# SafeRL-Lab/Massive-MARL-Benchmark

Hardware: AMD Instinct MI355X
Metric: env-steps/sec (whole node), TenAnt 4096 envs/GPU, PPO rollout (higher is better)
Workload: dtype f32 (policy-layer products: fp32 operands as 2 row-scaled fp16 planes (kept to 2^-22), 3 f16 MFMA products, fp32 accumulation; error vs float64 <= the exact-fp32 MFMA kernel's, see policy_layers_error_vs_f64); 1 GPU; TenAnt num_envs=4096 per GPU, PPO rollout: ActorCritic MLP [1024,1024,512]x2 (fp32) + fused sim step (dt 0.0166, 2 substeps) + RolloutStorage + GAE every 8 steps; envs_per_gpu=4096, global_envs=4096, parallelism=env-sharded x1, no data-path collective, hipgraph=True, refresh_in_graph=True, rollouts_per_graph=1, fused_act_and_bound_slots=True, obs_planes_from_step_kernel=True, policy_head_in_step_kernel=True, critic_stream=True, critic_deferred=False, finite=True, resets_total=97569

## Files before the change

include/mms.h:

```cpp
#ifndef MMS_H
#define MMS_H

#include <stdint.h>

#ifdef __cplusplus
extern "C" {
#endif

#define MMS_ABI_VERSION 4
#define MMS_DR_FLOATS 33

enum mms_task { MMS_TASK_TEN_ANT = 0, MMS_TASK_ONE_ANT = 1, MMS_TASK_MULTI_INGENUITY = 2,
                MMS_TASK_MULTI_ANT_CIRCLE = 3 };
enum mms_dtype { MMS_F32 = 0, MMS_I64 = 1, MMS_I32 = 2, MMS_U8 = 3 };

typedef struct mms_model {
    float torso_mass, torso_ixx, torso_izz, torso_radius;
    float leg_mass, leg_ia, leg_it;
    float foot_mass, foot_ia, foot_it;
    float limb_radius, leg_len, foot_len;
    float hip_pos[4][3];
    float limb_dir[4][3];
    float ankle_axis[4][3];
    float dof_lower[8], dof_upper[8], dof_init[8], gear[8];
// ... 176 lines not shown
#define MMS_H32_BYTES(rows, K) ((size_t)(rows) * (size_t)(((K) + 31) / 32) * 128)

int mms_split_planes16_group(int device, int32_t groups, int64_t rows, int32_t K, int32_t x_pitch, const float* const* x, void* const* planes,
                             float* const* scale, float* const* inv, int32_t nchains, int32_t L, const float* const* chain,
                             float* const* chain_scale, float* const* chain_inv, float* const* stat, float eps, void* hip_stream);

int mms_split_planes16_cat(int device, int64_t rows, int32_t K0, int32_t pitch0, const float* x0, int32_t K1, int32_t pitch1, const float* x1,
                           void* planes, float* scale, float* inv, int32_t nchains, int32_t L, const float* chain, float* chain_scale,
                           float* chain_inv, void* hip_stream);

int mms_weight_planes16_group(int device, int32_t groups, const int64_t* N, const int32_t* K, const float* const* w, void* const* planes,
                              float* const* scale, float* const* inv, float* const* l1, void* hip_stream);
int mms_chain_refresh16(int device, int32_t nchains, int32_t L, const float* const* l1, const float* const* bias, const int32_t* n,
                        float* chain, float bound0, int64_t rows, float* chain_scale, float* chain_inv, void* hip_stream);

int mms_linear_group_act_split16(int device, int32_t groups, int64_t M, int32_t N, int32_t K, const void* const* x, const void* const* w,
                                 const float* const* b, void* const* y, const float* const* x_inv, const float* const* w_inv,
                                 const float* const* y_scale, int32_t act, int32_t out_mode, const float* const* ln_s,
                                 const float* const* ln_stat_in, float* const* ln_part_out, const float* const* head_w, float* const* head_part,
                                 const int32_t* head_dims, void* hip_stream);

int mms_fold_planes16_group(int device, int32_t groups, const int64_t* N, const int32_t* K, const float* const* w, const float* const* gamma,
                            const float* const* beta, const float* const* bias, void* const* planes, float* const* inv, float* const* s,
                            float* const* c, float* const* rb, float* const* wt, void* hip_stream);
int mms_fold_scales16_group(int device, int32_t groups, const float* const* rb, const int32_t* n, int64_t M, float* const* scale1,
                            float* const* ysc, float* const* yinv, void* hip_stream);

int mms_row_stats_chan_group(int device, int32_t groups, int64_t M, int32_t slots, const float* const* part, float* const* stat, float eps,
                             void* hip_stream);

// ... 53 lines not shown
```

massive_marl_benchmark_amd/_lib.py:

```python
import ctypes
import os

from .model import MmsConfig, MmsTensor

_HERE = os.path.dirname(os.path.abspath(__file__))
LIB_PATH = os.environ.get("MMS_LIB", os.path.join(_HERE, "lib", "libmms.so"))
LIB_CPU_PATH = os.path.join(_HERE, "lib", "libmms_cpu.so")
_lib = None
_lib_cpu = None

SYMBOLS = ["mms_create", "mms_destroy", "mms_get_tensor", "mms_step", "mms_post_step", "mms_reset_all", "mms_set_state",
           "mms_bind_obs_out", "mms_bind_obs_planes16", "mms_bind_actions", "mms_bind_policy_head", "mms_set_dr", "mms_set_obs_outputs", "mms_bind_rollout_out", "mms_ppo_act", "mms_ppo_heads_act", "mms_sac_heads_act", "mms_q_heads_backup", "mms_det_heads_act_group", "mms_q_heads_backup_group", "mms_linear2_act", "mms_linear_group_act", "mms_split_planes", "mms_split_planes_group", "mms_linear_group_act_split", "mms_split_planes16_group", "mms_split_planes16_cat", "mms_weight_planes16_group", "mms_chain_refresh16", "mms_fold_planes16_group", "mms_fold_scales16_group", "mms_linear_group_act_split16", "mms_row_stats_chan_group", "mms_marl_heads_finish", "mms_row_stats_group", "mms_row_moments_group", "mms_layernorm_group", "mms_marl_heads_act", "mms_marl_views", "mms_gae_ppo", "mms_adv_normalize", "mms_gae_ppo_normalized", "mms_layer_clock_probe", "mms_gae_marl", "mms_gae_marl_agents", "mms_mlp_grad", "mms_mlp_grad_rop", "mms_ln_mlp_grad", "mms_ln_mlp_jvp", "mms_ppo_loss", "mms_marl_ppo_loss",
           "mms_last_error", "mms_abi_version"]


class MmsError(RuntimeError):
    pass


def _bind(path):
    L = ctypes.CDLL(path)
    vp, ci, c64, cf = ctypes.c_void_p, ctypes.c_int, ctypes.c_int64, ctypes.c_float
    L.mms_create.argtypes = [ctypes.POINTER(MmsConfig), ctypes.POINTER(vp)]
    L.mms_destroy.argtypes = [vp]
    L.mms_get_tensor.argtypes = [vp, ctypes.c_char_p, ctypes.POINTER(MmsTensor)]
    L.mms_step.argtypes = [vp, vp]
    L.mms_post_step.argtypes = [vp, vp]
# ... 14 lines not shown
    L.mms_q_heads_backup.argtypes = [ci, c64, ctypes.c_int32, vp, vp, vp, vp, vp, vp, vp, vp, vp, vp, vp, cf, cf, vp, vp]
    L.mms_det_heads_act_group.argtypes = [ci, ctypes.c_int32, c64, ctypes.c_int32, ctypes.c_int32, ctypes.c_int32, vp, vp, vp, vp, cf, ctypes.c_uint64, vp, c64, vp, c64, vp, c64, vp]
    L.mms_q_heads_backup_group.argtypes = [ci, ctypes.c_int32, c64, ctypes.c_int32, vp, vp, vp, vp, vp, vp, cf, vp, vp]
    L.mms_linear2_act.argtypes = [ci, c64, ctypes.c_int32, ctypes.c_int32, vp, vp, vp, vp, vp, vp, vp, vp, ctypes.c_int32, vp]
    L.mms_linear_group_act.argtypes = [ci, ctypes.c_int32, c64, ctypes.c_int32, ctypes.c_int32, vp, vp, vp, vp, ctypes.c_int32, vp, vp, vp, vp]
    L.mms_split_planes.argtypes = [ci, c64, ctypes.c_int32, ctypes.c_int32, vp, vp, vp]
    L.mms_split_planes_group.argtypes = [ci, ctypes.c_int32, c64, ctypes.c_int32, ctypes.c_int32, vp, vp, vp]
    L.mms_linear_group_act_split.argtypes = [ci, ctypes.c_int32, c64, ctypes.c_int32, ctypes.c_int32, vp, vp, vp, vp, ctypes.c_int32, ctypes.c_int32,
                                             vp, vp, vp, vp, vp, vp, vp]
    L.mms_split_planes16_group.argtypes = [ci, ctypes.c_int32, c64, ctypes.c_int32, ctypes.c_int32, vp, vp, vp, vp, ctypes.c_int32, ctypes.c_int32, vp, vp, vp, vp, cf, vp]
    L.mms_split_planes16_cat.argtypes = [ci, c64, ctypes.c_int32, ctypes.c_int32, vp, ctypes.c_int32, ctypes.c_int32, vp, vp, vp, vp, ctypes.c_int32, ctypes.c_int32, vp, vp, vp, vp]
    L.mms_weight_planes16_group.argtypes = [ci, ctypes.c_int32, vp, vp, vp, vp, vp, vp, vp, vp]
    L.mms_fold_planes16_group.argtypes = [ci, ctypes.c_int32, vp, vp, vp, vp, vp, vp, vp, vp, vp, vp, vp, vp, vp]
    L.mms_fold_scales16_group.argtypes = [ci, ctypes.c_int32, vp, vp, c64, vp, vp, vp, vp]
    L.mms_chain_refresh16.argtypes = [ci, ctypes.c_int32, ctypes.c_int32, vp, vp, vp, vp, cf, c64, vp, vp, vp]
    L.mms_linear_group_act_split16.argtypes = [ci, ctypes.c_int32, c64, ctypes.c_int32, ctypes.c_int32, vp, vp, vp, vp, vp, vp, vp, ctypes.c_int32, ctypes.c_int32,
                                               vp, vp, vp, vp, vp, vp, vp]
    L.mms_row_stats_chan_group.argtypes = [ci, ctypes.c_int32, c64, ctypes.c_int32, vp, vp, cf, vp]
    L.mms_marl_heads_finish.argtypes = [ci, ctypes.c_int32, c64, ctypes.c_int32, vp, vp, vp, vp, vp, vp, vp, vp, vp, vp, ctypes.c_uint64, c64, cf, vp]
    L.mms_row_moments_group.argtypes = [ci, ctypes.c_int32, c64, ctypes.c_int32, ctypes.c_int32, vp, vp, cf, vp]
    L.mms_row_stats_group.argtypes = [ci, ctypes.c_int32, c64, ctypes.c_int32, ctypes.c_int32, vp, vp, cf, vp]
    L.mms_layernorm_group.argtypes = [ci, ctypes.c_int32, c64, ctypes.c_int32, ctypes.c_int32, ctypes.c_int32, vp, vp, vp, vp, cf, vp]
    L.mms_marl_heads_act.argtypes = [ci, ctypes.c_int32, c64, ctypes.c_int32, vp, vp, vp, vp, vp, vp, vp, vp, vp, vp, vp, ctypes.c_uint64, c64, cf, vp]
    L.mms_marl_views.argtypes = [ci, vp, vp, c64, ctypes.c_int32, ctypes.c_int32, ctypes.c_int32, vp]
    L.mms_gae_ppo.argtypes = [ci, vp, vp, vp, vp, vp, vp, vp, ctypes.c_int32, c64, cf, cf, vp]
    L.mms_adv_normalize.argtypes = [ci, vp, vp, c64, vp]
    L.mms_gae_ppo_normalized.argtypes = [ci, vp, vp, vp, vp, vp, vp, vp, ctypes.c_int32, c64, cf, cf, vp]
    L.mms_layer_clock_probe.argtypes = [ci, vp, ctypes.c_int32]
    L.mms_gae_marl.argtypes = [ci, vp, vp, vp, vp, ctypes.c_int32, c64, cf, cf, ctypes.c_int32, vp, vp, vp]
    L.mms_gae_marl_agents.argtypes = [ci, vp, vp, vp, vp, ctypes.c_int32, c64, ctypes.c_int32, cf, cf, ctypes.c_int32, vp, vp, vp]
# ... 54 lines not shown
```

massive_marl_benchmark_amd/algorithms/rl/ppo/module.py:

```python
import ctypes
import math

import numpy as np
import torch
import torch.nn as nn

from .... import _lib


def get_activation(act_name):
    table = {"elu": nn.ELU, "selu": nn.SELU, "relu": nn.ReLU, "crelu": nn.ReLU, "lrelu": nn.LeakyReLU, "tanh": nn.Tanh,
             "sigmoid": nn.Sigmoid}
    if act_name not in table:
        print("invalid activation function!")
        return None
    return table[act_name]()


def _mlp(in_dim, hidden, out_dim, activation):
    layers, d = [], in_dim
    for h in hidden:
        layers += [nn.Linear(d, h), activation]
        d = h
    layers.append(nn.Linear(d, out_dim))
# ... 164 lines not shown
    def _chain(self, st, members):
        o0, Lh = st["slices"][members[0]]
        if Lh == 0:
            return None, 0
        for j, g in enumerate(members):
            assert st["slices"][g] == (o0 + 2 * Lh * j, Lh), "networks that share an input must be adjacent and equally deep"
        return st["bounds"][o0: o0 + 2 * Lh * len(members)], Lh

    def refresh(self):
        dev = self.log_std.device
        vers, addrs = self._param_tags()
        if self._addr_tag is not None and self._addr_tag != (addrs, str(dev)):
            self._h16, self._wplanes, self._split_bufs, self._calls, self._sample_calls = None, None, None, None, None
            self._head_wt = None
        self._addr_tag, self._ver_tag = (addrs, str(dev)), vers
        if self._head_wt is not None:
            self._fill_head_tiles()
        st = self._h16
        if st is not None:
            stream = _lib.for_device(st["dev"])[2]
            for fn, args, what in st["calls"]:
                _lib.check(fn(*args, stream), None, what, st["L"])
            covered = set()
            for (members, rows, scale), (_, cs, ci, alias) in st["given"].items():
                ca = self._chain_args(st, members)
                if ca is None or alias:
                    continue
                _lib.check(st["L"].mms_chain_refresh16(st["idx"], *ca, 16384.0 / scale, rows, ctypes.c_void_p(cs.data_ptr()), ctypes.c_void_p(ci.data_ptr()), stream),
                           None, "mms_chain_refresh16", st["L"])
                covered.update(members)
            depths = {Lh for _, Lh in st["slices"]}
            rest = [tuple(range(len(st["recs"])))] if len(depths) == 1 else [(g,) for g in range(len(st["recs"]))]
            for grp in rest:
                if not set(grp) <= covered:
                    ca = self._chain_args(st, grp)
                    if ca is not None:
                        _lib.check(st["L"].mms_chain_refresh16(st["idx"], *ca, 0.0, 0, None, None, stream), None, "mms_chain_refresh16", st["L"])
        if self._wplanes:
            for key in list(self._wplanes):
                tag, planes, lin = self._wplanes[key]
                if self.split_format == "bf16x3":
                    self._weight_planes(lin, *_lib.for_device(lin.weight.device), force=True)
                else:
                    self._wplanes[key] = (None, planes, lin)

    def _head_tiles(self):
        if self._head_wt is None:
            last = self.actor[-1]
            A, H = last.out_features, last.in_features
            nct = (A + 15) // 16
            pad = torch.zeros(nct * 16, H, device=last.weight.device, dtype=torch.float32)
            tiles = torch.empty(nct * (H // 4) * 64, device=last.weight.device, dtype=torch.float32)
            self._head_wt = (pad, tiles)
            self._fill_head_tiles()
        return self._head_wt[1]

    def _fill_head_tiles(self):
        pad, tiles = self._head_wt
        last = self.actor[-1]
# ... 348 lines not shown
            p = lambda t: ctypes.c_void_p(t.data_ptr())
            h, M = x.contiguous(), x.shape[0]
            if self._split_applies(M, lin[:-1], networks=1) and h.data_ptr() % 16 == 0:
                h = self._split_hidden([lin[:-1]], [h], "value", obs_planes)[0]
            else:
                key = (M, str(x.device))
                if self._value_bufs is None or self._value_bufs[0] != key:
                    self._value_bufs = (key, [torch.empty(M, l.out_features, device=x.device) for l in lin[:-1]])
                for l, y in zip(lin[:-1], self._value_bufs[1]):
                    _lib.check(L.mms_linear2_act(idx, M, l.out_features, l.in_features, p(h), p(l.weight.detach()), p(l.bias.detach()), p(y),
                                                 None, None, None, None, 1, stream), None, "mms_linear2_act", L)
                    h = y
            out = torch.empty(M, 1, device=x.device)
            one = lambda t: (ctypes.c_void_p * 1)(t.data_ptr())
            w, b = lin[-1].weight.detach(), lin[-1].bias.detach()
            _lib.check(L.mms_marl_heads_act(idx, 1, M, lin[-1].in_features, one(h), one(w), one(w), one(w), one(b), (ctypes.c_int32 * 1)(1), None,
                                            one(out), None, None, None, 0, 0, -1.0, stream), None, "mms_marl_heads_act", L)
            return out

    def act_inference(self, observations):
        return self.actor(observations)

    def evaluate(self, observations, states, actions):
        mean = self.actor(observations)
        scale_log = 2.0 * self.log_std
        z = (actions - mean) * torch.exp(-scale_log)
        log_prob = (-0.5 * z * z - scale_log - 0.5 * math.log(2.0 * math.pi)).sum(-1)
        entropy = (0.5 + 0.5 * math.log(2.0 * math.pi) + scale_log).sum(-1).expand(mean.shape[0])
        value = self.critic(states if self.asymmetric else observations)
        return log_prob, entropy, value, mean, self.log_std.repeat(mean.shape[0], 1)
# ... 10 lines not shown
```

massive_marl_benchmark_amd/csrc/cpu/mms_cpu.cpp:

```cpp
#include <math.h>
#include <stdio.h>
#include <stdlib.h>
#include <string.h>

#include <string>
#include <vector>

#include "../mms_host.h"
#include "../rollout_lane.h"
#include "../ppo_loss_lane.h"
#include "../marl_loss_lane.h"
#include "../q_lane.h"
#include "../maddpg_lane.h"
#include "../sac_lane.h"
#include "lane_step.h"

#define MMS_API extern "C" __attribute__((visibility("default")))

struct mms_engine : mms_host_state {};

template <typename T> static T* buf(mms_engine* e, const char* name) { return (T*)find(e, name)->ptr; }

MMS_API int mms_abi_version(void) { return MMS_ABI_VERSION; }
MMS_API const char* mms_last_error(mms_handle h) { return h ? h->err.c_str() : g_error.c_str(); }
// ... 636 lines not shown
        }
        chain[2 * e] = m;
        chain[2 * e + 1] = b;
    }
    for (int c = 0; c < nchains && rows > 0; c++) {
        float bound = bound0;
        for (int l = 0; l < L; l++) {
            bound = (chain[((size_t)c * L + l) * 2] * bound + chain[((size_t)c * L + l) * 2 + 1]) * 1.001f;
            float sc, iv;
            pow2_scale(bound, sc, iv);
            for (int64_t r = 0; r < rows; r++) {
                chain_scale[((size_t)c * L + l) * rows + r] = sc;
                chain_inv[((size_t)c * L + l) * rows + r] = iv;
            }
        }
    }
    return 0;
}

MMS_API int mms_fold_planes16_group(int device, int32_t groups, const int64_t* N, const int32_t* K, const float* const* w, const float* const* gamma,
                                    const float* const* beta, const float* const* bias, void* const* planes, float* const* inv, float* const* s_out,
                                    float* const* c_out, float* const* rb, float* const* wt, void*) {
    if (cpu_only(device)) return 1;
    if (refused(check_fold_planes16_group(groups, N, K, w, planes, inv))) return 1;
    for (int g = 0; g < groups; g++) {
        const int Kg = K[g], KC = (Kg + 31) / 32;
        const float* gm = gamma ? gamma[g] : nullptr;
        const float* bt = beta ? beta[g] : nullptr;
        uint16_t* out = planes ? (uint16_t*)planes[g] : nullptr;
#pragma omp parallel for schedule(static)
// ... 644 lines not shown
```

massive_marl_benchmark_amd/csrc/mms_api.hip:

```cpp
#include <hip/hip_runtime.h>
#include <stdio.h>
#include <stdlib.h>

#include "mms_host.h"
#include "policy_args.h"
#include "step_args.h"
#include "trpo_plan.h"
#include "ln_mlp_plan.h"
#include "maddpg_args.h"

namespace mms {
hipError_t launch_step(const StepArgs& a, int task, hipStream_t stream);
bool step_layout_takes_head(int task, int num_envs, int num_agents, int packing);
hipError_t launch_gae_ppo(const float*, const uint8_t*, const float*, const float*, float*, float*, double*, int, int64_t, float, float, hipStream_t);
hipError_t launch_adv_normalize(float*, const double*, int64_t, hipStream_t);
hipError_t launch_gae_ppo_normalized(const float*, const uint8_t*, const float*, const float*, float*, float*, double*, int, int64_t, float, float, hipStream_t);
hipError_t launch_gae_marl(const float*, const float*, const float*, float*, int, int64_t, float, float, int, const float*, const float*, hipStream_t);
hipError_t launch_marl_views(const float*, float*, int64_t, int, int, int, hipStream_t);
hipError_t launch_gae_marl_agents(const float*, const float*, const float*, float*, int, int64_t, int, float, float, int, const float*, const float*, hipStream_t);
hipError_t launch_ppo_act(const float*, const float*, const float*, uint64_t, int64_t*, int64_t, int, float*, float*, float*, float*, float*, float*, int64_t, int, hipStream_t);
hipError_t launch_ppo_head_act(const float*, const float*, const float*, int, const float*, const float*, const float*, const float*, int, const float*, uint64_t,
                               int64_t*, int64_t, int, float*, float*, float*, float*, float*, float*, int64_t, int, hipStream_t);
hipError_t launch_sac_head_act(const float*, int, const float*, const float*, const float*, const float*, float, float, int, uint64_t, int64_t*, int64_t,
                               float*, float*, float*, float*, float*, float*, int64_t, int, hipStream_t);
// ... 454 lines not shown
    return 0;
}

__attribute__((visibility("default"))) int mms_chain_refresh16(int device, int32_t nchains, int32_t L, const float* const* l1, const float* const* bias,
                                                               const int32_t* n, float* chain, float bound0, int64_t rows, float* chain_scale,
                                                               float* chain_inv, void* s) {
    MMS_DEV(device)
    if (refused(check_chain_refresh16(nchains, L, l1, n, chain, bound0, rows, chain_scale, chain_inv))) return 1;
    mms::ChainRefreshArgs a = {};
    for (int e = 0; e < nchains * L; e++) { a.l1[e] = l1[e]; a.bias[e] = bias ? bias[e] : nullptr; a.n[e] = n[e]; }
    a.chain = chain; a.nchains = nchains; a.L = L; a.bound0 = bound0; a.rows = rows; a.chain_scale = chain_scale; a.chain_inv = chain_inv;
    MMS_FREE(mms::launch_chain_refresh16(a, (hipStream_t)s));
    return 0;
}

__attribute__((visibility("default"))) int mms_fold_planes16_group(int device, int32_t groups, const int64_t* N, const int32_t* K, const float* const* w,
                                                                   const float* const* gamma, const float* const* beta, const float* const* bias,
                                                                   void* const* planes, float* const* inv, float* const* s_out, float* const* c_out,
                                                                   float* const* rb, float* const* wt, void* s) {
    MMS_DEV(device)
    if (refused(check_fold_planes16_group(groups, N, K, w, planes, inv))) return 1;
    mms::FoldPlanesArgs a = {};
    for (int g = 0; g < groups; g++) {
        a.w[g] = w[g];
        a.gamma[g] = gamma ? gamma[g] : nullptr; a.beta[g] = beta ? beta[g] : nullptr; a.bias[g] = bias ? bias[g] : nullptr;
        a.planes[g] = planes ? planes[g] : nullptr; a.inv[g] = inv ? inv[g] : nullptr;
        a.s[g] = s_out ? s_out[g] : nullptr; a.c[g] = c_out ? c_out[g] : nullptr; a.rb[g] = rb ? rb[g] : nullptr; a.wt[g] = wt ? wt[g] : nullptr;
        a.rows_g[g] = N[g]; a.K_g[g] = K[g];
    }
    MMS_FREE(mms::launch_fold_planes16(a, groups, (hipStream_t)s));
// ... 266 lines not shown
```

massive_marl_benchmark_amd/csrc/mms_host.h:

```cpp
#pragma once
#include <math.h>
#include <stdint.h>
#include <string.h>

#include <string>
#include <vector>

#include "../../include/mms.h"

namespace mms {
constexpr int kMlpMaxLayers = 8;
constexpr int64_t kMlpMaxRows = 65535 * 32 / 128 * 128;
}

struct mms_buffer {
    const char* name;
    void* ptr;
    int64_t shape[4];
    int ndim;
    int dtype;
    size_t bytes;
    int64_t row_bytes;
};

// ... 481 lines not shown
        if (!w[g] || !planes[g] || !scale[g] || !inv[g] || (addr(planes[g]) & 15) != 0 || (addr(w[g]) & 3) != 0 || (addr(inv[g]) & 15) != 0)
            return "mms_weight_planes16_group: null or misaligned pointer in a group (planes and inv 16-byte aligned)";
    }
    return {};
}

static inline std::string check_chain_refresh16(int32_t nchains, int32_t L, const float* const* l1, const int32_t* n, const float* chain, float bound0,
                                                int64_t rows, const float* chain_scale, const float* chain_inv) {
    if (nchains < 1 || L < 1 || (int64_t)nchains * L > MMS_MAX_GROUPS || !l1 || !n || !chain || rows < 0 || (rows > 0 && (!chain_scale || !chain_inv || !(bound0 >= 0.f))))
        return "mms_chain_refresh16: bad arguments (nchains, L >= 1, nchains * L <= " + std::to_string(MMS_MAX_GROUPS) + "; rows > 0 needs chain_scale, chain_inv, bound0 >= 0)";
    for (int e = 0; e < nchains * L; e++)
        if (!l1[e] || n[e] < 0) return "mms_chain_refresh16: null pointer or negative count in an entry";
    return {};
}

static inline std::string check_fold_planes16_group(int32_t groups, const int64_t* N, const int32_t* K, const float* const* w, void* const* planes,
                                                    float* const* inv) {
    std::string bad = check_groups("mms_fold_planes16_group", groups);
    if (!bad.empty()) return bad;
    if (!N || !K || !w) return "mms_fold_planes16_group: bad arguments (null array)";
    for (int g = 0; g < groups; g++) {
        if (N[g] < 0 || K[g] <= 0) return "mms_fold_planes16_group: bad shape in a group (N >= 0, K > 0)";
        if (!w[g] || (planes && planes[g] && (!inv || !inv[g])) || (planes && (addr(planes[g]) & 15) != 0))
            return "mms_fold_planes16_group: null or misaligned pointer in a group (planes 16-byte aligned and with inv)";
    }
    return {};
}

static inline std::string check_fold_scales16_group(int32_t groups, const float* const* rb, const int32_t* n, int64_t M) {
    std::string bad = check_groups("mms_fold_scales16_group", groups);
// ... 175 lines not shown
```

massive_marl_benchmark_amd/csrc/policy_args.h:

```cpp
#pragma once
#include <hip/hip_runtime.h>
#include <stdint.h>

#include "../../include/mms.h"

namespace mms {

constexpr int kMaxGroups = MMS_MAX_GROUPS;

struct LinearArgs {
    const float* x[kMaxGroups];
    const float* w[kMaxGroups];
    const float* b[kMaxGroups];
    float* y[kMaxGroups];
    int M, N, K;
    int act;
    const float* s[kMaxGroups];
    const float* stat_in[kMaxGroups];
    float* part_out[kMaxGroups];
};

struct RowStatsArgs {
    const float* part[kMaxGroups];
    float* stat[kMaxGroups];
// ... 126 lines not shown
    int nchains, L;
};

struct ChainRefreshArgs {
    const float* l1[kMaxGroups];
    const float* bias[kMaxGroups];
    int n[kMaxGroups];
    float* chain;
    int nchains, L;
    float bound0;
    int64_t rows;
    float* chain_scale;
    float* chain_inv;
};

struct FoldPlanesArgs {
    const float* w[kMaxGroups];
    const float* gamma[kMaxGroups];
    const float* beta[kMaxGroups];
    const float* bias[kMaxGroups];
    void* planes[kMaxGroups];
    float* inv[kMaxGroups];
    float* s[kMaxGroups];
    float* c[kMaxGroups];
    float* rb[kMaxGroups];
    float* wt[kMaxGroups];
    int64_t rows_g[kMaxGroups];
    int K_g[kMaxGroups];
};

struct FoldScalesArgs {
    const float* rb[kMaxGroups];
    float* scale1[kMaxGroups];
    float* ysc[kMaxGroups];
    float* yinv[kMaxGroups];
    int n[kMaxGroups];
    int64_t M;
};

hipError_t launch_fold_planes16(const FoldPlanesArgs& a, int groups, hipStream_t s);
hipError_t launch_fold_scales16(const FoldScalesArgs& a, int groups, hipStream_t s);
hipError_t launch_split16_planes_group(const Split16PlanesArgs& a, int groups, hipStream_t s);
hipError_t launch_split16_planes_cat(const Split16CatArgs& a, hipStream_t s);
hipError_t launch_chain_refresh16(const ChainRefreshArgs& a, hipStream_t s);
hipError_t launch_linear_split16(const Split16LinearArgs& a, int groups, hipStream_t s);
void set_split16_clock_probe(uint64_t* out, int slots);
hipError_t launch_linear_act(const LinearArgs& a, int groups, hipStream_t s);
hipError_t launch_row_stats_chan(const RowStatsArgs& a, int groups, hipStream_t s);
hipError_t launch_marl_heads_finish(const HeadsFinishArgs& a, int groups, hipStream_t s);
hipError_t launch_split_planes_group(const SplitPlanesArgs& a, int groups, hipStream_t s);
hipError_t launch_linear_split(const SplitLinearArgs& a, int groups, hipStream_t s);
hipError_t launch_split_planes(const float* x, void* planes, int64_t rows, int K, int x_pitch, hipStream_t s);
hipError_t launch_row_stats(const RowStatsArgs& a, int groups, hipStream_t s);
hipError_t launch_layernorm(const LayerNormArgs& a, int groups, hipStream_t s);
hipError_t launch_marl_heads(const HeadsArgs& a, int groups, hipStream_t s);

}
```

massive_marl_benchmark_amd/csrc/policy_kernels.hip:

```cpp
#include <hip/hip_runtime.h>
#include <stdint.h>
#include <stdlib.h>

#include "mms_lane.h"
#include "policy_args.h"

namespace mms {

typedef float f32x16 __attribute__((ext_vector_type(16)));

constexpr int kTM = 128, kTN = 128;

__device__ __forceinline__ float apply_act(float v, int act) {
    if (act == 1) return (v > 0.f) ? v : (expf(v) - 1.f);
    if (act == 2) return fmaxf(v, 0.f);
    if (act == 3) return 1.f - 2.f / (__expf(2.f * v) + 1.f);
    return v;
}


constexpr int kBK = 32, kPitch = kBK + 4;
constexpr size_t kLinearLds = (size_t)2 * 2 * 128 * kPitch * sizeof(float);

template <int MI>
// ... 475 lines not shown
        float* out = a.out[g] + row * a.out_pitch[g];
        if (a.std[g] == nullptr) {
            if (lane < A) out[lane] = mine;
            continue;
        }
        const int64_t c = a.counters[g] ? a.counters[g][row] : 0;
        if (lane < A) {
            const float z = rand_normal(a.seed + (uint64_t)g, (uint64_t)(a.row_offset + row), (uint64_t)c, (uint32_t)lane);
            out[lane] = mine + sd * z;
            if (a.logp[g]) a.logp[g][row * a.out_pitch[g] + lane] = fmaf(-0.5f * z, z, -lk);
        }
        if (lane == 0 && a.counters[g]) a.counters[g][row] = c + 1;
    }
}

__global__ void __launch_bounds__(256) row_stats_kernel(RowStatsArgs a) {
    const int g = blockIdx.y;
    const int64_t row = (int64_t)blockIdx.x * 256 + threadIdx.x;
    if (row >= a.M) return;
    const float2* part = reinterpret_cast<const float2*>(a.part[g]);
    float sum = 0.f, sq = 0.f;
    for (int k = 0; k < a.slots; k++) {
        const float2 p = part[(size_t)k * a.M + row];
        sum += p.x;
        sq += p.y;
    }
    const float inv = 1.0f / (float)a.width;
    const float mean = sum * inv;
    const float var = fmaxf(sq * inv - mean * mean, 0.f);
    reinterpret_cast<float2*>(a.stat[g])[row] = make_float2(mean, 1.0f / sqrtf(var + a.eps));
// ... 122 lines not shown
```

massive_marl_benchmark_amd/csrc/split16_kernels.hip:

```cpp
#include <hip/hip_runtime.h>
#include <stdint.h>
#include <stdlib.h>

#include <type_traits>

#include "policy_args.h"

namespace mms {

typedef _Float16 f16x8 __attribute__((ext_vector_type(8)));
typedef _Float16 f16x4 __attribute__((ext_vector_type(4)));
typedef float f32x4 __attribute__((ext_vector_type(4)));
typedef uint32_t u32x4_16 __attribute__((ext_vector_type(4)));

#ifndef MMS_S16_AUX_X
#define MMS_S16_AUX_X 0
#endif
#ifndef MMS_S16_AUX_W
#define MMS_S16_AUX_W 0
#endif
#ifndef MMS_S16_STAMP
#define MMS_S16_STAMP 0
#endif
#ifndef MMS_S16_EXP
// ... 254 lines not shown
        float bound = a.bound0;
        for (int l = 0; l < a.L; l++) {
            bound = (s_chain[2 * (c * a.L + l)] * bound + s_chain[2 * (c * a.L + l) + 1]) * 1.001f;
            float sc, iv;
            pow2_scale(bound, sc, iv);
            a.chain_scale[((size_t)c * a.L + l) * a.rows + row] = sc;
            a.chain_inv[((size_t)c * a.L + l) * a.rows + row] = iv;
        }
    }
}

hipError_t launch_chain_refresh16(const ChainRefreshArgs& a, hipStream_t s) {
    if (a.nchains * a.L == 0) return hipSuccess;
    const unsigned blocks = a.rows > 0 ? (unsigned)((a.rows + 255) / 256) : 1u;
    hipLaunchKernelGGL(chain_refresh16_kernel, dim3(blocks), dim3(256), 0, s, a);
    return hipGetLastError();
}

template <int MT>
struct Geom16 {
    static constexpr int TM = 64 * MT, TN = 128;
    static constexpr int XBYTES = TM * kChunk16, WBYTES = TN * kChunk16, BUF = XBYTES + WBYTES;
    static constexpr int NDMA = BUF / 1024 / 8;
    static constexpr int NX = TM / 64;
    static constexpr int SCRATCH = 8 * 16 * (2 * kChunk16 + 16);
    static constexpr bool SCRATCH_IN_BUF = BUF >= SCRATCH;
    static constexpr int HW_OFF = 3 * BUF + (SCRATCH_IN_BUF ? 0 : SCRATCH);
    static constexpr size_t LDS = (size_t)HW_OFF + 16 * 128 * 4;
};

// ... 537 lines not shown
```

Before: 29.34 million env-steps/s.

## Fuse policy weight-plane refresh, chain bounds and head tiling into one kernel

Replaces the sequence of per-update refresh launches (weight fp16 plane split, chain-bound refresh, head tile fill) with a single kernel. A last-block atomic counter lets the final block compute the chain bounds and per-row scales. It also adds a dedicated wave-per-row value-head dot-product kernel in place of the generic multi-head act kernel for the critic output. The aim is fewer launches and less launch and graph overhead, at the cost of a grid-wide atomic counter that must be reset correctly and a more complex fused kernel.

```diff
diff --git a/include/mms.h b/include/mms.h
--- a/include/mms.h
+++ b/include/mms.h
@@ -214,6 +214,16 @@
 int mms_chain_refresh16(int device, int32_t nchains, int32_t L, const float* const* l1, const float* const* bias, const int32_t* n,
                         float* chain, float bound0, int64_t rows, float* chain_scale, float* chain_inv, void* hip_stream);
 
+#define MMS_REFRESH_MAX_SETS 8
+int mms_policy_refresh16(int device, int32_t groups, const int64_t* N, const int32_t* K, const float* const* w, void* const* planes,
+                         float* const* scale, float* const* inv, float* const* l1, const float* const* bias, int32_t nets, int32_t L,
+                         float* chain, int32_t nsets, const int32_t* set_first, const int32_t* set_nchains, const float* set_bound0,
+                         const int64_t* set_rows, float* const* set_scale, float* const* set_inv, const float* head_w, int32_t A,
+                         int32_t H, float* head_tiles, void* workspace, void* hip_stream);
+
+int mms_value_rows(int device, int64_t M, int32_t H, int64_t h_pitch, const float* h, const float* w, const float* b, float* y,
+                   void* hip_stream);
+
 int mms_linear_group_act_split16(int device, int32_t groups, int64_t M, int32_t N, int32_t K, const void* const* x, const void* const* w,
                                  const float* const* b, void* const* y, const float* const* x_inv, const float* const* w_inv,
                                  const float* const* y_scale, int32_t act, int32_t out_mode, const float* const* ln_s,
diff --git a/massive_marl_benchmark_amd/_lib.py b/massive_marl_benchmark_amd/_lib.py
--- a/massive_marl_benchmark_amd/_lib.py
+++ b/massive_marl_benchmark_amd/_lib.py
@@ -10,7 +10,7 @@
 _lib_cpu = None
 
 SYMBOLS = ["mms_create", "mms_destroy", "mms_get_tensor", "mms_step", "mms_post_step", "mms_reset_all", "mms_set_state",
-           "mms_bind_obs_out", "mms_bind_obs_planes16", "mms_bind_actions", "mms_bind_policy_head", "mms_set_dr", "mms_set_obs_outputs", "mms_bind_rollout_out", "mms_ppo_act", "mms_ppo_heads_act", "mms_sac_heads_act", "mms_q_heads_backup", "mms_det_heads_act_group", "mms_q_heads_backup_group", "mms_linear2_act", "mms_linear_group_act", "mms_split_planes", "mms_split_planes_group", "mms_linear_group_act_split", "mms_split_planes16_group", "mms_split_planes16_cat", "mms_weight_planes16_group", "mms_chain_refresh16", "mms_fold_planes16_group", "mms_fold_scales16_group", "mms_linear_group_act_split16", "mms_row_stats_chan_group", "mms_marl_heads_finish", "mms_row_stats_group", "mms_row_moments_group", "mms_layernorm_group", "mms_marl_heads_act", "mms_marl_views", "mms_gae_ppo", "mms_adv_normalize", "mms_gae_ppo_normalized", "mms_layer_clock_probe", "mms_gae_marl", "mms_gae_marl_agents", "mms_mlp_grad", "mms_mlp_grad_rop", "mms_ln_mlp_grad", "mms_ln_mlp_jvp", "mms_ppo_loss", "mms_marl_ppo_loss",
+           "mms_bind_obs_out", "mms_bind_obs_planes16", "mms_bind_actions", "mms_bind_policy_head", "mms_set_dr", "mms_set_obs_outputs", "mms_bind_rollout_out", "mms_ppo_act", "mms_ppo_heads_act", "mms_sac_heads_act", "mms_q_heads_backup", "mms_det_heads_act_group", "mms_q_heads_backup_group", "mms_linear2_act", "mms_linear_group_act", "mms_split_planes", "mms_split_planes_group", "mms_linear_group_act_split", "mms_split_planes16_group", "mms_split_planes16_cat", "mms_weight_planes16_group", "mms_chain_refresh16", "mms_policy_refresh16", "mms_value_rows", "mms_fold_planes16_group", "mms_fold_scales16_group", "mms_linear_group_act_split16", "mms_row_stats_chan_group", "mms_marl_heads_finish", "mms_row_stats_group", "mms_row_moments_group", "mms_layernorm_group", "mms_marl_heads_act", "mms_marl_views", "mms_gae_ppo", "mms_adv_normalize", "mms_gae_ppo_normalized", "mms_layer_clock_probe", "mms_gae_marl", "mms_gae_marl_agents", "mms_mlp_grad", "mms_mlp_grad_rop", "mms_ln_mlp_grad", "mms_ln_mlp_jvp", "mms_ppo_loss", "mms_marl_ppo_loss",
            "mms_last_error", "mms_abi_version"]
 
 
@@ -55,6 +55,8 @@
     L.mms_fold_planes16_group.argtypes = [ci, ctypes.c_int32, vp, vp, vp, vp, vp, vp, vp, vp, vp, vp, vp, vp, vp]
     L.mms_fold_scales16_group.argtypes = [ci, ctypes.c_int32, vp, vp, c64, vp, vp, vp, vp]
     L.mms_chain_refresh16.argtypes = [ci, ctypes.c_int32, ctypes.c_int32, vp, vp, vp, vp, cf, c64, vp, vp, vp]
+    L.mms_policy_refresh16.argtypes = [ci, ctypes.c_int32] + [vp] * 8 + [ctypes.c_int32, ctypes.c_int32, vp, ctypes.c_int32] + [vp] * 6 + [vp, ctypes.c_int32, ctypes.c_int32, vp, vp, vp]
+    L.mms_value_rows.argtypes = [ci, c64, ctypes.c_int32, c64, vp, vp, vp, vp, vp]
     L.mms_linear_group_act_split16.argtypes = [ci, ctypes.c_int32, c64, ctypes.c_int32, ctypes.c_int32, vp, vp, vp, vp, vp, vp, vp, ctypes.c_int32, ctypes.c_int32,
                                                vp, vp, vp, vp, vp, vp, vp]
     L.mms_row_stats_chan_group.argtypes = [ci, ctypes.c_int32, c64, ctypes.c_int32, vp, vp, cf, vp]
diff --git a/massive_marl_benchmark_amd/algorithms/rl/ppo/module.py b/massive_marl_benchmark_amd/algorithms/rl/ppo/module.py
--- a/massive_marl_benchmark_amd/algorithms/rl/ppo/module.py
+++ b/massive_marl_benchmark_amd/algorithms/rl/ppo/module.py
@@ -1,11 +1,15 @@
 import ctypes
 import math
+import os
 
 import numpy as np
 import torch
 import torch.nn as nn
 
 from .... import _lib
+
+_ONE_REFRESH = os.environ.get("MMS_ONE_REFRESH", "1") != "0"
+_VALUE_ROWS = os.environ.get("MMS_VALUE_ROWS", "1") != "0"
 
 
 def get_activation(act_name):
@@ -202,10 +206,13 @@
             self._h16, self._wplanes, self._split_bufs, self._calls, self._sample_calls = None, None, None, None, None
             self._head_wt = None
         self._addr_tag, self._ver_tag = (addrs, str(dev)), vers
-        if self._head_wt is not None:
+        st = self._h16
+        one = self._refresh_one(st) if st is not None and _ONE_REFRESH else None
+        if one is not None:
+            _lib.check(st["L"].mms_policy_refresh16(*one, _lib.for_device(st["dev"])[2]), None, "mms_policy_refresh16", st["L"])
+        elif self._head_wt is not None:
             self._fill_head_tiles()
-        st = self._h16
-        if st is not None:
+        if st is not None and one is None:
             stream = _lib.for_device(st["dev"])[2]
             for fn, args, what in st["calls"]:
                 _lib.check(fn(*args, stream), None, what, st["L"])
@@ -231,6 +238,38 @@
                     self._weight_planes(lin, *_lib.for_device(lin.weight.device), force=True)
                 else:
                     self._wplanes[key] = (None, planes, lin)
+
+    def _refresh_one(self, st):
+        head = self._head_wt[1].data_ptr() if self._head_wt is not None else None
+        sets = [(k, v) for k, v in st["given"].items() if not v[3]]
+        tag = (head, tuple(k for k, _ in sets))
+        hit = st.get("one")
+        if hit is not None and hit[0] == tag:
+            return hit[1]
+        recs = st["recs"]
+        Lh = st["slices"][0][1]
+        ok = (len(recs) >= 1 and Lh >= 1 and all(s == (2 * Lh * j, Lh) for j, s in enumerate(st["slices"])) and len(sets) <= 8
+              and all(k[0] == tuple(range(k[0][0], k[0][0] + len(k[0]))) for k, _ in sets))
+        last = self.actor[-1]
+        if head is not None:
+            ok = ok and last.weight.is_contiguous() and last.in_features % 4 == 0 and last.weight.data_ptr() % 16 == 0 and last.weight.device == st["dev"]
+        args = None
+        if ok:
+            flat = [r for rs in recs for r in rs]
+            arr = lambda ts: (ctypes.c_void_p * len(ts))(*[t.data_ptr() for t in ts])
+            i32 = lambda vs: (ctypes.c_int32 * max(len(vs), 1))(*vs)
+            if "count" not in st:
+                st["count"] = torch.zeros(1, dtype=torch.int32, device=st["dev"])
+            args = (st["idx"], len(flat), (ctypes.c_int64 * len(flat))(*[r["N"] for r in flat]), i32([r["K"] for r in flat]),
+                    arr([r["lin"].weight for r in flat]), arr([r["planes"] for r in flat]), arr([r["scale"] for r in flat]),
+                    arr([r["inv"] for r in flat]), arr([r["l1"] for r in flat]), arr([r["lin"].bias for r in flat]), len(recs), Lh,
+                    ctypes.c_void_p(st["bounds"].data_ptr()), len(sets), i32([k[0][0] for k, _ in sets]), i32([len(k[0]) for k, _ in sets]),
+                    (ctypes.c_float * max(len(sets), 1))(*[16384.0 / k[2] for k, _ in sets]), (ctypes.c_int64 * max(len(sets), 1))(*[k[1] for k, _ in sets]),
+                    arr([v[1] for _, v in sets]) if sets else None, arr([v[2] for _, v in sets]) if sets else None,
+                    ctypes.c_void_p(last.weight.data_ptr()) if head is not None else None, last.out_features, last.in_features,
+                    ctypes.c_void_p(head) if head is not None else None, ctypes.c_void_p(st["count"].data_ptr()))
+        st["one"] = (tag, args)
+        return args
 
     def _head_tiles(self):
         if self._head_wt is None:
@@ -609,6 +648,9 @@
             out = torch.empty(M, 1, device=x.device)
             one = lambda t: (ctypes.c_void_p * 1)(t.data_ptr())
             w, b = lin[-1].weight.detach(), lin[-1].bias.detach()
+            if _VALUE_ROWS:
+                _lib.check(L.mms_value_rows(idx, M, lin[-1].in_features, h.stride(0), p(h), p(w), p(b), p(out), stream), None, "mms_value_rows", L)
+                return out
             _lib.check(L.mms_marl_heads_act(idx, 1, M, lin[-1].in_features, one(h), one(w), one(w), one(w), one(b), (ctypes.c_int32 * 1)(1), None,
                                             one(out), None, None, None, 0, 0, -1.0, stream), None, "mms_marl_heads_act", L)
             return out
diff --git a/massive_marl_benchmark_amd/csrc/cpu/mms_cpu.cpp b/massive_marl_benchmark_amd/csrc/cpu/mms_cpu.cpp
--- a/massive_marl_benchmark_amd/csrc/cpu/mms_cpu.cpp
+++ b/massive_marl_benchmark_amd/csrc/cpu/mms_cpu.cpp
@@ -674,6 +674,64 @@
                 chain_inv[((size_t)c * L + l) * rows + r] = iv;
             }
         }
+    }
+    return 0;
+}
+
+MMS_API int mms_policy_refresh16(int device, int32_t groups, const int64_t* N, const int32_t* K, const float* const* w, void* const* planes,
+                                 float* const* scale, float* const* inv, float* const* l1, const float* const* bias, int32_t nets, int32_t L,
+                                 float* chain, int32_t nsets, const int32_t* set_first, const int32_t* set_nchains, const float* set_bound0,
+                                 const int64_t* set_rows, float* const* set_scale, float* const* set_inv, const float* head_w, int32_t A,
+                                 int32_t H, float* head_tiles, void* workspace, void*) {
+    if (cpu_only(device)) return 1;
+    if (refused(check_policy_refresh16(groups, N, K, w, planes, scale, inv, l1, nets, L, chain, nsets, set_first, set_nchains, set_bound0, set_rows,
+                                       set_scale, set_inv, head_w, A, H, head_tiles, workspace))) return 1;
+    if (mms_weight_planes16_group(device, groups, N, K, w, planes, scale, inv, l1, nullptr)) return 1;
+    const float* el1[MMS_MAX_GROUPS];
+    const float* ebias[MMS_MAX_GROUPS];
+    int32_t en[MMS_MAX_GROUPS];
+    for (int e = 0; e < nets * L; e++) {
+        const int g = (e / L) * (L + 1) + e % L;
+        el1[e] = l1[g]; ebias[e] = bias ? bias[g] : nullptr; en[e] = (int32_t)N[g];
+    }
+    if (mms_chain_refresh16(device, nets, L, el1, ebias, en, chain, 0.f, 0, nullptr, nullptr, nullptr)) return 1;
+    for (int s = 0; s < nsets; s++)
+        for (int c = 0; c < set_nchains[s]; c++) {
+            float bound = set_bound0[s];
+            for (int l = 0; l < L; l++) {
+                const int e = (set_first[s] + c) * L + l;
+                bound = (chain[2 * e] * bound + chain[2 * e + 1]) * 1.001f;
+                float sc, iv;
+                pow2_scale(bound, sc, iv);
+                for (int64_t r = 0; r < set_rows[s]; r++) {
+                    set_scale[s][((size_t)c * L + l) * set_rows[s] + r] = sc;
+                    set_inv[s][((size_t)c * L + l) * set_rows[s] + r] = iv;
+                }
+            }
+        }
+    if (head_w) {
+        const int HQ = H / 4, nct = (A + 15) / 16;
+        for (int ct = 0; ct < nct; ct++)
+            for (int kq = 0; kq < HQ; kq++)
+                for (int i = 0; i < 16; i++)
+                    for (int j = 0; j < 4; j++) {
+                        const int o = ct * 16 + i;
+                        head_tiles[(((size_t)ct * HQ + kq) * 16 + i) * 4 + j] = o < A ? head_w[(size_t)o * H + kq * 4 + j] : 0.f;
+                    }
+    }
+    return 0;
+}
+
+MMS_API int mms_value_rows(int device, int64_t M, int32_t H, int64_t h_pitch, const float* h, const float* w, const float* b, float* y, void*) {
+    if (cpu_only(device)) return 1;
+    if (h_pitch == 0) h_pitch = H;
+    if (refused(check_value_rows(M, H, h_pitch, h, w, b, y))) return 1;
+#pragma omp parallel for schedule(static)
+    for (int64_t m = 0; m < M; m++) {
+        float p = 0.f;
+        for (int k = 0; k < H; k++) p += h[m * h_pitch + k] * w[k];
+        p += b[0];
+        y[m] = p;
     }
     return 0;
 }
diff --git a/massive_marl_benchmark_amd/csrc/mms_api.hip b/massive_marl_benchmark_amd/csrc/mms_api.hip
--- a/massive_marl_benchmark_amd/csrc/mms_api.hip
+++ b/massive_marl_benchmark_amd/csrc/mms_api.hip
@@ -492,6 +492,43 @@
     return 0;
 }
 
+__attribute__((visibility("default"))) int mms_policy_refresh16(int device, int32_t groups, const int64_t* N, const int32_t* K, const float* const* w,
+                                                                void* const* planes, float* const* scale, float* const* inv, float* const* l1,
+                                                                const float* const* bias, int32_t nets, int32_t L, float* chain, int32_t nsets,
+                                                                const int32_t* set_first, const int32_t* set_nchains, const float* set_bound0,
+                                                                const int64_t* set_rows, float* const* set_scale, float* const* set_inv,
+                                                                const float* head_w, int32_t A, int32_t H, float* head_tiles, void* workspace, void* s) {
+    MMS_DEV(device)
+    if (refused(check_policy_refresh16(groups, N, K, w, planes, scale, inv, l1, nets, L, chain, nsets, set_first, set_nchains, set_bound0, set_rows,
+                                       set_scale, set_inv, head_w, A, H, head_tiles, workspace))) return 1;
+    mms::PolicyRefreshArgs a = {};
+    for (int g = 0; g < groups; g++) {
+        a.w[g] = w[g]; a.planes[g] = planes[g]; a.scale[g] = scale[g]; a.inv[g] = inv[g]; a.l1[g] = l1[g];
+        a.bias[g] = bias ? bias[g] : nullptr;
+        a.rows_g[g] = N[g]; a.K_g[g] = K[g];
+    }
+    a.groups = groups; a.nets = nets; a.L = L; a.chain = chain; a.nsets = nsets;
+    for (int i = 0; i < nsets; i++) {
+        a.set_first[i] = set_first[i]; a.set_nch[i] = set_nchains[i]; a.set_bound0[i] = set_bound0[i]; a.set_rows[i] = set_rows[i];
+        a.set_scale[i] = set_scale[i]; a.set_inv[i] = set_inv[i];
+    }
+    a.head_w = head_w; a.head_tiles = head_w ? head_tiles : nullptr; a.A = head_w ? A : 0; a.H = head_w ? H : 0;
+    a.counter = (uint32_t*)workspace;
+    MMS_FREE(mms::launch_policy_refresh16(a, (hipStream_t)s));
+    return 0;
+}
+
+__attribute__((visibility("default"))) int mms_value_rows(int device, int64_t M, int32_t H, int64_t h_pitch, const float* h, const float* w,
+                                                          const float* b, float* y, void* s) {
+    MMS_DEV(device)
+    if (h_pitch == 0) h_pitch = H;
+    if (refused(check_value_rows(M, H, h_pitch, h, w, b, y))) return 1;
+    mms::ValueRowsArgs a = {};
+    a.h = h; a.w = w; a.b = b; a.y = y; a.M = M; a.h_pitch = h_pitch; a.H = H;
+    MMS_FREE(mms::launch_value_rows(a, (hipStream_t)s));
+    return 0;
+}
+
 __attribute__((visibility("default"))) int mms_fold_planes16_group(int device, int32_t groups, const int64_t* N, const int32_t* K, const float* const* w,
                                                                    const float* const* gamma, const float* const* beta, const float* const* bias,
                                                                    void* const* planes, float* const* inv, float* const* s_out, float* const* c_out,
diff --git a/massive_marl_benchmark_amd/csrc/mms_host.h b/massive_marl_benchmark_amd/csrc/mms_host.h
--- a/massive_marl_benchmark_amd/csrc/mms_host.h
+++ b/massive_marl_benchmark_amd/csrc/mms_host.h
@@ -519,6 +519,41 @@
     return {};
 }
 
+static inline std::string check_policy_refresh16(int32_t groups, const int64_t* N, const int32_t* K, const float* const* w, void* const* planes,
+                                                 float* const* scale, float* const* inv, float* const* l1, int32_t nets, int32_t L, const float* chain,
+                                                 int32_t nsets, const int32_t* set_first, const int32_t* set_nchains, const float* set_bound0,
+                                                 const int64_t* set_rows, float* const* set_scale, float* const* set_inv, const float* head_w, int32_t A,
+                                                 int32_t H, const float* head_tiles, const void* workspace) {
+    std::string bad = check_groups("mms_policy_refresh16", groups);
+    if (!bad.empty()) return bad;
+    if (!workspace || (addr(workspace) & 3) != 0) return "mms_policy_refresh16: null or misaligned workspace (4 bytes of zeroed device memory)";
+    if (nets < 1 || L < 1 || (int64_t)nets * (L + 1) != groups)
+        return "mms_policy_refresh16: mismatched counts (nets >= 1, L >= 1, groups == nets * (L + 1))";
+    if (!N || !K || !w || !planes || !scale || !inv || !l1 || !chain) return "mms_policy_refresh16: bad arguments (null array)";
+    int64_t items = 0;
+    for (int g = 0; g < groups; g++) {
+        if (N[g] < 0 || N[g] > 0x7fffffff || K[g] <= 0) return "mms_policy_refresh16: bad shape in a group (0 <= N < 2^31, K > 0)";
+        if (!w[g] || !planes[g] || !scale[g] || !inv[g] || !l1[g] || (addr(planes[g]) & 15) != 0 || (addr(w[g]) & 3) != 0 || (addr(inv[g]) & 15) != 0)
+            return "mms_policy_refresh16: null or misaligned pointer in a group (planes and inv 16-byte aligned)";
+        items += N[g];
+    }
+    if (items > 0x3fffffff) return "mms_policy_refresh16: bad shape (too many rows in all)";
+    if (nsets < 0 || nsets > MMS_REFRESH_MAX_SETS || (nsets > 0 && (!set_first || !set_nchains || !set_bound0 || !set_rows || !set_scale || !set_inv)))
+        return "mms_policy_refresh16: bad arguments (0 <= nsets <= " + std::to_string(MMS_REFRESH_MAX_SETS) + ", every set array given)";
+    for (int s = 0; s < nsets; s++)
+        if (set_first[s] < 0 || set_nchains[s] < 1 || set_first[s] + set_nchains[s] > nets || set_rows[s] <= 0 || !(set_bound0[s] >= 0.f) || !set_scale[s] || !set_inv[s])
+            return "mms_policy_refresh16: bad set (chains inside 0..nets, rows > 0, bound0 >= 0, set_scale, set_inv)";
+    if (head_w && (!head_tiles || A < 1 || H < 4 || H % 4 != 0 || (int64_t)((A + 15) / 16) * H > 0x3fffffff || (addr(head_w) & 15) != 0 || (addr(head_tiles) & 15) != 0))
+        return "mms_policy_refresh16: bad head (A >= 1, H a multiple of 4, head_w and head_tiles 16-byte aligned)";
+    return {};
+}
+
+static inline std::string check_value_rows(int64_t M, int32_t H, int64_t h_pitch, const float* h, const float* w, const float* b, const float* y) {
+    if (M < 0 || H < 1 || H > 1024 || h_pitch < H) return "mms_value_rows: bad arguments (M >= 0, 1 <= H <= 1024, h_pitch >= H)";
+    if (!h || !w || !b || !y || ((addr(h) | addr(w) | addr(b) | addr(y)) & 3) != 0) return "mms_value_rows: null or misaligned pointer";
+    return {};
+}
+
 static inline std::string check_fold_planes16_group(int32_t groups, const int64_t* N, const int32_t* K, const float* const* w, void* const* planes,
                                                     float* const* inv) {
     std::string bad = check_groups("mms_fold_planes16_group", groups);
diff --git a/massive_marl_benchmark_amd/csrc/policy_args.h b/massive_marl_benchmark_amd/csrc/policy_args.h
--- a/massive_marl_benchmark_amd/csrc/policy_args.h
+++ b/massive_marl_benchmark_amd/csrc/policy_args.h
@@ -164,6 +164,41 @@
     float* chain_inv;
 };
 
+constexpr int kMaxRefreshSets = 8;
+struct PolicyRefreshArgs {
+    const float* w[kMaxGroups];
+    void* planes[kMaxGroups];
+    float* scale[kMaxGroups];
+    float* inv[kMaxGroups];
+    float* l1[kMaxGroups];
+    const float* bias[kMaxGroups];
+    int64_t rows_g[kMaxGroups];
+    int K_g[kMaxGroups];
+    int item_end[kMaxGroups];
+    int groups, nets, L;
+    float* chain;
+    int nsets;
+    int set_first[kMaxRefreshSets], set_nch[kMaxRefreshSets];
+    float set_bound0[kMaxRefreshSets];
+    int64_t set_rows[kMaxRefreshSets];
+    float* set_scale[kMaxRefreshSets];
+    float* set_inv[kMaxRefreshSets];
+    const float* head_w;
+    float* head_tiles;
+    int A, H;
+    int split_items, items;
+    uint32_t* counter;
+};
+
+struct ValueRowsArgs {
+    const float* h;
+    const float* w;
+    const float* b;
+    float* y;
+    int64_t M, h_pitch;
+    int H;
+};
+
 struct FoldPlanesArgs {
     const float* w[kMaxGroups];
     const float* gamma[kMaxGroups];
@@ -193,6 +228,8 @@
 hipError_t launch_split16_planes_group(const Split16PlanesArgs& a, int groups, hipStream_t s);
 hipError_t launch_split16_planes_cat(const Split16CatArgs& a, hipStream_t s);
 hipError_t launch_chain_refresh16(const ChainRefreshArgs& a, hipStream_t s);
+hipError_t launch_policy_refresh16(PolicyRefreshArgs& a, hipStream_t s);
+hipError_t launch_value_rows(const ValueRowsArgs& a, hipStream_t s);
 hipError_t launch_linear_split16(const Split16LinearArgs& a, int groups, hipStream_t s);
 void set_split16_clock_probe(uint64_t* out, int slots);
 hipError_t launch_linear_act(const LinearArgs& a, int groups, hipStream_t s);
diff --git a/massive_marl_benchmark_amd/csrc/policy_kernels.hip b/massive_marl_benchmark_amd/csrc/policy_kernels.hip
--- a/massive_marl_benchmark_amd/csrc/policy_kernels.hip
+++ b/massive_marl_benchmark_amd/csrc/policy_kernels.hip
@@ -513,6 +513,42 @@
     }
 }
 
+constexpr int kValueRows = 4;
+__global__ void __launch_bounds__(256) value_rows_kernel(ValueRowsArgs a) {
+    const int lane = threadIdx.x & 63, wave = threadIdx.x >> 6;
+    const int H = a.H;
+    const int64_t row0 = ((int64_t)blockIdx.x * 4 + wave) * kValueRows;
+    if (row0 >= a.M) return;
+    float w[kLnPerLane], v[kValueRows][kLnPerLane];
+#pragma unroll
+    for (int i = 0; i < kLnPerLane; i++) w[i] = (lane + 64 * i < H) ? a.w[lane + 64 * i] : 0.f;
+#pragma unroll
+    for (int r = 0; r < kValueRows; r++) {
+        const int64_t row = row0 + r < a.M ? row0 + r : a.M - 1;
+        const float* __restrict__ h = a.h + row * a.h_pitch;
+#pragma unroll
+        for (int i = 0; i < kLnPerLane; i++) v[r][i] = (lane + 64 * i < H) ? h[lane + 64 * i] : 0.f;
+    }
+    const float bias = a.b[0];
+#pragma unroll
+    for (int r = 0; r < kValueRows; r++) {
+        float p = (lane < H) ? v[r][0] * w[0] : 0.f;
+#pragma unroll
+        for (int i = 1; i < kLnPerLane; i++) if (lane + 64 * i < H) p = __builtin_fmaf(v[r][i], w[i], p);
+        p = wave_all_sum(p);
+        float mine = p;
+        mine += bias;
+        if (lane == 0 && row0 + r < a.M) a.y[row0 + r] = mine;
+    }
+}
+
+hipError_t launch_value_rows(const ValueRowsArgs& a, hipStream_t s) {
+    if (a.M == 0) return hipSuccess;
+    const int64_t per_block = 4 * kValueRows;
+    hipLaunchKernelGGL(value_rows_kernel, dim3((unsigned)((a.M + per_block - 1) / per_block)), dim3(256), 0, s, a);
+    return hipGetLastError();
+}
+
 __global__ void __launch_bounds__(256) row_stats_kernel(RowStatsArgs a) {
     const int g = blockIdx.y;
     const int64_t row = (int64_t)blockIdx.x * 256 + threadIdx.x;
diff --git a/massive_marl_benchmark_amd/csrc/split16_kernels.hip b/massive_marl_benchmark_amd/csrc/split16_kernels.hip
--- a/massive_marl_benchmark_amd/csrc/split16_kernels.hip
+++ b/massive_marl_benchmark_amd/csrc/split16_kernels.hip
@@ -292,6 +292,156 @@
     if (a.nchains * a.L == 0) return hipSuccess;
     const unsigned blocks = a.rows > 0 ? (unsigned)((a.rows + 255) / 256) : 1u;
     hipLaunchKernelGGL(chain_refresh16_kernel, dim3(blocks), dim3(256), 0, s, a);
+    return hipGetLastError();
+}
+
+template <bool ALIGNED>
+__global__ void __launch_bounds__(1024) policy_refresh16_kernel(PolicyRefreshArgs a) {
+    __shared__ float s_chain[2 * kMaxGroups];
+    __shared__ int s_last;
+    const int lane = threadIdx.x & 63, wave = __builtin_amdgcn_readfirstlane(threadIdx.x >> 6);
+    const int item = blockIdx.x * 4 + (wave >> 2), wv = wave & 3;
+    if (item < a.split_items) {
+        int g = 0;
+        while (item >= a.item_end[g]) g++;
+        const int bx = item - (g ? a.item_end[g - 1] : 0);
+        const float* __restrict__ x = a.w[g];
+        uint8_t* __restrict__ out = reinterpret_cast<uint8_t*>(a.planes[g]);
+        const int K = a.K_g[g], KC = (K + 31) / 32;
+        const int64_t rows = a.rows_g[g];
+        int P = 1;
+        while (P < KC * 4 && P < 64) P <<= 1;
+        const int sub = lane & (P - 1), rpw = 64 / P;
+        const int64_t row_raw = ((int64_t)bx * 4 + wv) * rpw + lane / P;
+        const bool live = row_raw < rows;
+        const int64_t row = live ? row_raw : rows - 1;
+        const float* src = x + row * (int64_t)K;
+        const int pieces = KC * 4;
+        auto load8 = [&](int p, float* v) {
+            const int k0 = p * 8;
+            if (ALIGNED && k0 + 8 <= K) {
+                const float4 q0 = *reinterpret_cast<const float4*>(src + k0), q1 = *reinterpret_cast<const float4*>(src + k0 + 4);
+                v[0] = q0.x; v[1] = q0.y; v[2] = q0.z; v[3] = q0.w; v[4] = q1.x; v[5] = q1.y; v[6] = q1.z; v[7] = q1.w;
+            } else {
+#pragma unroll
+                for (int j = 0; j < 8; j++) v[j] = (k0 + j < K) ? src[k0 + j] : 0.f;
+            }
+        };
+        float big = 0.f, asum = 0.f;
+        for (int p = sub; p < pieces; p += P) {
+            float v[8];
+            load8(p, v);
+#pragma unroll
+            for (int j = 0; j < 8; j++) { big = fmaxf(big, fabsf(v[j])); asum += fabsf(v[j]); }
+        }
+        for (int m = P >> 1; m >= 1; m >>= 1) {
+            big = fmaxf(big, __shfl_xor(big, m, 64));
+            asum += __shfl_xor(asum, m, 64);
+        }
+        float scale, inv;
+        pow2_scale(big, scale, inv);
+        for (int p = sub; p < pieces; p += P) {
+            float v[8];
+            load8(p, v);
+            f16x8 hi, lo;
+#pragma unroll
+            for (int j = 0; j < 8; j++) {
+                const float t = v[j] * scale;
+                hi[j] = (_Float16)t;
+                lo[j] = (_Float16)((t - (float)hi[j]) * kLoScale);
+            }
+            if (live) {
+                uint8_t* dst = out + (row * KC + (p >> 2)) * (int64_t)kChunk16 + (p & 3) * 16;
+                *reinterpret_cast<f16x8*>(dst) = hi;
+                *reinterpret_cast<f16x8*>(dst + 64) = lo;
+            }
+        }
+        if (sub == 0 && live) {
+            a.scale[g][row] = scale;
+            a.inv[g][row] = inv;
+            a.l1[g][row] = asum;
+        }
+    } else if (item < a.items) {
+        const int HQ = a.H >> 2, nf4 = ((a.A + 15) >> 4) * HQ * 16;
+        const int t = (item - a.split_items) * 256 + wv * 64 + lane;
+        if (t < nf4) {
+            const int i = t & 15, kq = (t >> 4) % HQ, ct = (t >> 4) / HQ;
+            const int j = ct * 16 + i;
+            float4 q = make_float4(0.f, 0.f, 0.f, 0.f);
+            if (j < a.A) q = *reinterpret_cast<const float4*>(a.head_w + (size_t)j * a.H + 4 * kq);
+            reinterpret_cast<float4*>(a.head_tiles)[t] = q;
+        }
+    }
+    asm volatile("s_waitcnt vmcnt(0)" ::: "memory");
+    __syncthreads();
+    if (threadIdx.x == 0) {
+        __builtin_amdgcn_fence(__ATOMIC_RELEASE, "agent");
+        asm volatile("s_waitcnt vmcnt(0)" ::: "memory");
+        const uint32_t seen = __hip_atomic_fetch_add(a.counter, 1u, __ATOMIC_RELAXED, __HIP_MEMORY_SCOPE_AGENT);
+        const int last = seen == gridDim.x - 1;
+        if (last) {
+            __builtin_amdgcn_fence(__ATOMIC_ACQUIRE, "agent");
+            asm volatile("s_waitcnt vmcnt(0)" ::: "memory");
+        }
+        s_last = last;
+    }
+    __syncthreads();
+    if (!s_last) return;
+    const int L = a.L, E = a.nets * L;
+    for (int e = wave; e < E; e += 16) {
+        const int g = (e / L) * (L + 1) + e % L;
+        const float* __restrict__ l1 = a.l1[g];
+        const float* __restrict__ bias = a.bias[g];
+        const int n = (int)a.rows_g[g];
+        float m = 0.f, b = 0.f;
+        for (int i = lane; i < n; i += 64) {
+            m = fmaxf(m, l1[i]);
+            if (bias) b = fmaxf(b, fabsf(bias[i]));
+        }
+        for (int k = 32; k >= 1; k >>= 1) {
+            m = fmaxf(m, __shfl_xor(m, k, 64));
+            b = fmaxf(b, __shfl_xor(b, k, 64));
+        }
+        if (lane == 0) { s_chain[2 * e] = m; s_chain[2 * e + 1] = b; }
+    }
+    __syncthreads();
+    if ((int)threadIdx.x < 2 * E) a.chain[threadIdx.x] = s_chain[threadIdx.x];
+    for (int s = 0; s < a.nsets; s++) {
+        const int64_t rows = a.set_rows[s];
+        for (int c = 0; c < a.set_nch[s]; c++) {
+            float bound = a.set_bound0[s];
+            for (int l = 0; l < L; l++) {
+                const int e = (a.set_first[s] + c) * L + l;
+                bound = (s_chain[2 * e] * bound + s_chain[2 * e + 1]) * 1.001f;
+                float sc, iv;
+                pow2_scale(bound, sc, iv);
+                float* cs = a.set_scale[s] + ((size_t)c * L + l) * rows;
+                float* ci = a.set_inv[s] + ((size_t)c * L + l) * rows;
+                for (int64_t row = threadIdx.x; row < rows; row += 1024) { cs[row] = sc; ci[row] = iv; }
+            }
+        }
+    }
+    if (threadIdx.x == 0) __hip_atomic_store(a.counter, 0u, __ATOMIC_RELAXED, __HIP_MEMORY_SCOPE_AGENT);
+}
+
+hipError_t launch_policy_refresh16(PolicyRefreshArgs& a, hipStream_t s) {
+    bool aligned = true;
+    int items = 0;
+    for (int g = 0; g < a.groups; g++) {
+        aligned = aligned && (a.K_g[g] % 4) == 0 && (reinterpret_cast<uintptr_t>(a.w[g]) & 15) == 0;
+        const int KCg = (a.K_g[g] + 31) / 32;
+        int Pg = 1;
+        while (Pg < KCg * 4 && Pg < 64) Pg <<= 1;
+        const int64_t rpb = 4 * (64 / Pg);
+        items += (int)((a.rows_g[g] + rpb - 1) / rpb);
+        a.item_end[g] = items;
+    }
+    a.split_items = items;
+    if (a.head_w) items += (((a.A + 15) / 16) * (a.H / 4) * 16 + 255) / 256;
+    a.items = items;
+    const unsigned blocks = items > 0 ? (unsigned)((items + 3) / 4) : 1u;
+    if (aligned) hipLaunchKernelGGL(policy_refresh16_kernel<true>, dim3(blocks), dim3(1024), 0, s, a);
+    else hipLaunchKernelGGL(policy_refresh16_kernel<false>, dim3(blocks), dim3(1024), 0, s, a);
     return hipGetLastError();
 }
 
```

After: 29.14 million env-steps/s. Within noise of the previous version (-0.7%).
